# awslabs/dgl-ke

Measured on AMD Instinct MI355X. Metric: positive edges/sec (whole node), higher is better.
Workload: dtype f32

## Files before the change

dgl-ke_amd/csrc/kge_api.hip:

```cpp
#include <cmath>
#include <cstdarg>
#include <cstdio>
#include <cstring>
#include <new>
#include <algorithm>
#include "kge_common.hpp"
#include "kge_sampler_common.hpp"

namespace {

thread_local char g_err[512] = "";

int fail(int code, const char *fmt, ...) {
    va_list ap;
    va_start(ap, fmt);
    vsnprintf(g_err, sizeof(g_err), fmt, ap);
    va_end(ap);
    return code;
}

#define KGE_TRY(expr)                                                                  \
    do {                                                                               \
        const int rc_ = (expr);                                                        \
        if (rc_ != KGE_OK) return fail(rc_, "%s failed (%d) at %s:%d", #expr, rc_, __FILE__, __LINE__); \
// ... 211 lines not shown
        na.S = out;
        KGE_TRY(launch_neg_fwd_pair(na, s));
    }
    return KGE_OK;
}

int kge_score_neg_bwd(int model, int neg_head, const float *pos_side, const float *rel, const float *neg, const float *neg_score,
                      const float *dneg, int C, int chunk, int N, int d_e, int d_r, float gamma, float emb_init, float *g_pos_side,
                      float *g_rel, float *g_neg, void *ws, size_t ws_bytes, unsigned flags, void *stream) {
    if (int rc = check_model(model, d_e, d_r)) return rc;
    if (!pos_side || !rel || !neg || !dneg || !g_pos_side || !g_rel || !g_neg || !ws || C < 0 || chunk <= 0 || N <= 0)
        return fail(KGE_ERR_ARG, "kge_score_neg_bwd: bad argument");
    if (model == KGE_TRANSR) return no_modular_transr();
    if ((model == KGE_TRANSE_L2 || model == KGE_SIMPLE) && !neg_score)
        return fail(KGE_ERR_ARG, "kge_score_neg_bwd: TransE_l2 / SimplE need the forward scores");
    if (C == 0) return KGE_OK;
    hipStream_t s = (hipStream_t)stream;
    const int B = C * chunk;
    Carver cv(ws, ws_bytes); NegBufs w;
    const size_t need = carve_neg(cv, w, model, C, chunk, N, d_e);
    if (need > ws_bytes) return fail(KGE_ERR_WORKSPACE, "workspace too small: need %zu bytes", need);
    if (int rc = neg_prepare(model, neg_head, pos_side, rel, neg, C, chunk, N, d_e, d_r, gamma, emb_init, false, w, s)) return rc;
    const float *Wuse = dneg;
    if (model == KGE_TRANSE_L2 || model == KGE_SIMPLE) {
        const int64_t n = (int64_t)B * N;
        const dim3 grid((unsigned)((n + 255) / 256));
        if (model == KGE_TRANSE_L2) hipLaunchKernelGGL(l2_scale_kernel, grid, dim3(256), 0, s, dneg, neg_score, gamma, w.W, n);
        else hipLaunchKernelGGL(clamp_mask_kernel, grid, dim3(256), 0, s, dneg, neg_score, KGE_SIMPLE_CLAMP, w.W, n);
        Wuse = w.W;
    }
    bool gemm = use_mfma(model, d_e, N, flags);
    if (gemm) {
        GemmArgs g; fill_gemm(g, model, C, chunk, N, d_e, gamma, w.A, neg, nullptr);
        g.W = Wuse; g.GA = w.GA; g.GN = g_neg;
        const int rc = launch_neg_bwd_gemm(g, s);
        if (rc == KGE_ERR_ARG) gemm = false;
        else if (rc != KGE_OK) return fail(rc, "launch_neg_bwd_gemm failed (%d)", rc);
    }
    if (!gemm) {
        NegArgs na; fill_pair(na, model, C, chunk, N, d_e, gamma, w.A, neg, nullptr);
        na.W = Wuse; na.GA = w.GA; na.GN = g_neg;
        na.GNp = (flags & KGE_FLAG_TWO_PASS_PAIR) ? nullptr : w.GNp;
        KGE_TRY(launch_neg_bwd_pair(na, s));
    }
    if (model == KGE_RESCAL) {
        RescalMatvecArgs m{};
        m.B = B; m.D = d_e; m.rel = rel; m.z1 = w.GA; m.c1 = g_pos_side;
        KGE_TRY(launch_rescal_matvec(m, s));
        RescalOuterArgs o{};
        o.B = B; o.D = d_e; o.u = w.GA; o.v = pos_side; o.G = g_rel;
        KGE_TRY(launch_rescal_outer(o, s));
        return KGE_OK;
    }
    EdgeBwdArgs e;
    fill_edge_bwd(e, EdgeSrc{pos_side, nullptr, pos_side, nullptr, rel, nullptr}, model, B, d_e, d_r, neg_head, gamma,
                  rot_div_of(emb_init), nullptr, w.GA);
    e.GH = neg_head ? nullptr : g_pos_side;
    e.GT = neg_head ? g_pos_side : nullptr;
    e.GR = g_rel;
    KGE_TRY(launch_edge_bwd(e, s));
    return KGE_OK;
}

int kge_loss_fwd_bwd(int loss_genre, int adv, float adv_temp, int pairwise, float margin, const float *pos, const float *neg,
                     const float *w, int64_t B, int N, float *loss3, float *dpos, float *dneg, void *ws, size_t ws_bytes, void *stream) {
    if (int rc = check_loss(loss_genre, adv, pairwise)) return rc;
    if (!pos || !neg || !dpos || !dneg || !ws || B <= 0 || N <= 0)
// ... 386 lines not shown
    if (p.fold_loss) {
        LossArgs la; fill_step_loss(la); la.skip_pos = 1;
        KGE_TRY(launch_neg_fwd_gemm_with_edge_loss(g, ef, la, out->tickets, s));
    } else KGE_TRY(launch_neg_fwd_gemm_with_edge(g, ef, s, c.tail));
    return KGE_OK;
}

int Step::phase_fwd() {
    if (p.transr) {
    } else if (p.gemm) {
        if (int rc = fwd_gemm()) return rc;
    } else {
        if (c.co_update) KGE_TRY(launch_update(*c.co_update, s));
        if (p.merged_pair) {
            NegArgs nf = na;
            nf.nbase = tb->ent; nf.nidx = b->neg_ids;
            nf.xbase = tb->ent; nf.xidx = b->neg_head ? b->t_gid : b->h_gid; nf.rbase = tb->rel; nf.ridx = b->rel_ids;
            nf.asign = b->neg_head ? -1.f : 1.f;
            KGE_TRY(launch_neg_fwd_bcast_with_edge(nf, ef, s));
        } else KGE_TRY(launch_neg_fwd_pair(na, s));
    }
    if (p.fused_loss || p.fold_loss) return KGE_OK;
    LossArgs la; fill_step_loss(la);
    la.row_pos = p.want4 ? w.row_pos : nullptr;
    if (p.merged_fwd && p.is_l2) { la.l2_raw = 1; la.l2_chunk = b->chunk; la.asq = w.asq; la.bsq = w.bsq; }
    la.skip_pos = (p.pairwise || p.rescal || p.transr) ? 0 : 1; la.diag_chunk = p.nd ? b->chunk : 0;
    KGE_TRY(launch_loss(la, s));
    return KGE_OK;
}

int Step::bwd_neg_gemm() {
    g.W = w.S; g.w = b->edge_w; g.lp = lp;
    if (p.dense_bwd) { g.nbase = w.Bn; g.nidx = nullptr; }
    g.GA = w.GA; g.GN = GN;
    if (p.qfuse) {
        g.Q = w.GT; g.QP = w.GH; g.qc = b->neg_head ? 1.f : -1.f;
        if (!(out && out->g_rel)) g.GA = nullptr;
    }
    g.reg_coef = (p.reg && !p.nd) ? hp->reg_coef : 0.f; g.reg_norm = hp->reg_norm;
    g.row_neg = (p.fused_loss && p.want4) ? w.row_neg : nullptr;
    g.acc = p.fused_loss ? acc : nullptr;
    if (p.ew_bwd) {
        g.ew_ent = src.hbase; g.ew_rel = src.rbase; g.ew_h = src.hidx; g.ew_t = src.tidx; g.ew_r = src.ridx;
        g.ew_dpos = w.dP; g.ew_GH = w.GH; g.ew_GT = w.GT; g.ew_GR = GR;
        g.ew_reg_coef = p.reg ? hp->reg_coef : 0.f; g.ew_reg_norm = hp->reg_norm; g.ew_neg_head = b->neg_head;
        if (!(out && out->g_rel)) g.GA = nullptr;
    }
    if (c.co_prep) {
        const int rc = launch_neg_bwd_gemm_with_prep(g, *c.co_prep, s);
        if (rc == KGE_OK) return KGE_OK;
        if (rc != KGE_ERR_ARG) return fail(rc, "launch_neg_bwd_gemm_with_prep failed (%d)", rc);
    }
    KGE_TRY(launch_neg_bwd_gemm(g, s, c.tail));
    if (c.co_prep) KGE_TRY(launch_edge_fwd(*c.co_prep, s));
    return KGE_OK;
}

int Step::bwd_transr() {
    const int B = b->B, d_e = hp->d_e;
    KGE_TRY(launch_transr_bwd(tr, s));
    RescalMatvecArgs m{};
    m.B = B; m.D = d_e; m.Dc = hp->d_r; m.rel = tbx->proj; m.ridx = b->rel_ids;
    m.y1 = tr.SG; m.r1 = w.TR1; m.y2 = tr.DQ; m.r2 = w.TR2;
    KGE_TRY(launch_rescal_matvec(m, s));
    KGE_TRY(launch_rescal_axpy(w.dP, w.TR1, b->neg_head ? nullptr : w.TR2, B, d_e, w.GH, s, -1.f));
    KGE_TRY(launch_rescal_axpy(w.dP, w.TR1, b->neg_head ? w.TR2 : nullptr, B, d_e, w.GT, s, 1.f));
    if (p.nd) KGE_TRY(launch_nd_fold(GN, b->neg_head ? w.GH : w.GT, B, b->chunk, p.N, d_e, s));
// ... 693 lines not shown
```

dgl-ke_amd/csrc/kge_common.hpp:

```cpp
#pragma once
#include <hip/hip_runtime.h>
#include <stdint.h>
#include "../../include/kge_hip.h"

#define KGE_WAVE 64
#define KGE_BLOCK 256
#define KGE_WAVES_PER_BLOCK (KGE_BLOCK / KGE_WAVE)

typedef float f32x4 __attribute__((ext_vector_type(4)));


#ifdef KGE_TIMELINE
#define KGE_TL_PER_KERNEL 8192
static __device__ unsigned long long *kge_tl_buf = nullptr;
__device__ __forceinline__ void kge_tl_mark(int kid, int n) {
    asm volatile("s_waitcnt vmcnt(0) lgkmcnt(0)" ::: "memory");
    const int wid = (int)(blockIdx.x * (blockDim.x >> 6) + (threadIdx.x >> 6));
    if ((threadIdx.x & 63) == 0 && kge_tl_buf && wid < KGE_TL_PER_KERNEL)
        kge_tl_buf[((size_t)kid * KGE_TL_PER_KERNEL + wid) * 8 + 4 + n] = wall_clock64();
}
struct KgeTlScope {
    unsigned long long t0; int kid; int wid;
    __device__ __forceinline__ KgeTlScope(int kid_, int wid_) : kid(kid_), wid(wid_) { t0 = wall_clock64(); }
    __device__ __forceinline__ void mark(int n) { kge_tl_mark(kid, n); }
// ... 374 lines not shown
bool rank_gemm_supported(int model, int d_e);
size_t rank_gemm_mask_bytes(int rows, int64_t N);
int launch_rank_gemm(int model, const float *A, int rows, const float *nbase, const int64_t *nidx, int64_t N, int D, float gamma,
                     float clampv, const float *asq, const float *bsq, const float *P, void *mask, const int64_t *filt_ptr,
                     const int64_t *filt_ids, int64_t e0, int32_t *ranks, hipStream_t s);
struct ChunkCands {
    const int64_t *cand; int64_t n_cand, stride;
    const int64_t *own;
    int64_t n_ent, E; int chunk;
};
int launch_chunk_bsq(const ChunkCands &cc, int64_t c0, int rows, int64_t n_list, const float *ent, int D, float *bsq_own, float *bsq_c,
                     hipStream_t s);
int launch_rank_chunk_gemm(int model, const ChunkCands &cc, int64_t c0, int nch, const float *A, const float *asq, const float *P,
                           const float *ent, int D, float gamma, float clampv, const float *bsq_own, const float *bsq_c, int shared,
                           const int64_t *filt_ptr, const int64_t *filt_ids, int32_t *ranks, hipStream_t s);
int launch_chunk_ids(const ChunkCands &cc, int64_t cfirst, int nch, int m, int64_t ncols, int64_t *ids, hipStream_t s);
int launch_chunk_count(const ChunkCands &cc, int64_t cfirst, int nch, int m, int64_t ncols, const float *S, const float *P,
                       const int64_t *filt_ptr, const int64_t *filt_ids, int32_t *ranks, hipStream_t s);
int launch_rel_query(int model, const float *ent, const int64_t *h, const int64_t *t, int rows, int d_e, float *Q, float *qsq,
                     hipStream_t s);
int launch_rel_rotate_score(const float *ent, const float *rel, const int64_t *h, const int64_t *t, int rows, int64_t n_rel, int d_e,
                            float gamma, float rot_div, float *S, hipStream_t s);
int launch_rel_neg_rows(const float *rel, int64_t n_rel, int d_r, float *out, int64_t *ids, int64_t n_ids, hipStream_t s);
int launch_rel_count_t(const float *St, const float *P, int rows, int64_t N, const int64_t *filt_ptr, const int64_t *filt_ids,
                       int64_t e0, int32_t *ranks, hipStream_t s);
struct GemmArgs {
    int model, C, chunk, N, D;
    float gamma;
    const float *A;
    const float *nbase; const int64_t *nidx;
    const float *asq, *bsq;
    const float *xbase; const int64_t *xidx; const float *rbase; const int64_t *ridx; float asign;
    int lds_off;
    float *S;
    float clampv;
    float *PM, *PS, *PL;
    float *Sraw;
    float adv_temp;
    const float *W;
    const float *w;
    LossParams lp; int B;
    float *GA, *GN;
    float *Q; const float *QP; float qc;
    const float *ew_ent, *ew_rel; const int64_t *ew_h, *ew_t, *ew_r; const float *ew_dpos;
    float *ew_GH, *ew_GT, *ew_GR; float ew_reg_coef; int ew_reg_norm, ew_neg_head;
    float reg_coef; int reg_norm;
    float *row_neg;
    float *acc;
};
bool neg_mfma_supported(int model, int d_e, int N);
bool neg_gemm_fused_loss_supported(int chunk, int N);
int launch_neg_fwd_gemm(const GemmArgs &a, hipStream_t s);
int launch_neg_bwd_gemm(const GemmArgs &a, hipStream_t s, const SmpTail *tail = nullptr);
struct UpdateArgs;
int launch_neg_fwd_gemm_with_update(const GemmArgs &a, const UpdateArgs &u, hipStream_t s);
bool neg_fwd_gemm_with_edge_supported(int model, int d_e, int d_r);
int launch_neg_fwd_gemm_with_edge(const GemmArgs &a, const EdgeFwdArgs &e, hipStream_t s, const SmpTail *tail = nullptr);
struct LossArgs;
bool neg_fwd_loss_fold_supported(int model, int C, int chunk, int N, int d_e, int d_r);
int launch_neg_fwd_gemm_with_edge_loss(const GemmArgs &a, const EdgeFwdArgs &e, const LossArgs &la, int *tickets, hipStream_t s);
int launch_neg_bwd_gemm_with_prep(const GemmArgs &a, const EdgeFwdArgs &e, hipStream_t s);
int launch_neg_fwd_pair(const NegArgs &a, hipStream_t s);
int launch_neg_bwd_pair(const NegArgs &a, hipStream_t s);
struct RescalMatvecArgs {
    int B, D;
    int Dc;
// ... 91 lines not shown
```

dgl-ke_amd/csrc/kge_neg_gemm.hip:

```cpp
#include "kge_common.hpp"
#include "kge_update_body.hpp"
#include "kge_edge_fwd_body.hpp"
#include "kge_sampler_tail.hpp"
#include "kge_loss_body.hpp"

using namespace kge;
KGE_TL_DEFINE(gemm)

#define MFMA16(a, b, c) __builtin_amdgcn_mfma_f32_16x16x4f32((a), (b), (c), 0, 0, 0)
#define KGE_PIN_ACC(x, y) do { asm volatile("" : "+a"(x), "+a"(y) :: "memory"); __builtin_amdgcn_sched_barrier(0); } while (0)
#define KGE_ORDER() do { asm volatile("" ::: "memory"); __builtin_amdgcn_sched_barrier(0); } while (0)

bool neg_mfma_supported(int model, int d_e, int N) {
    (void)N;
    if (model != KGE_TRANSE_L2 && model != KGE_DISTMULT && model != KGE_COMPLEX && model != KGE_SIMPLE &&
        model != KGE_RESCAL) return false;
    return d_e % 4 == 0;
}

bool neg_gemm_fused_loss_supported(int chunk, int N) { return N <= 256 && chunk <= 768; }

static inline int check_launch_g() { return hipGetLastError() == hipSuccess ? KGE_OK : KGE_ERR_LAUNCH; }
__device__ __forceinline__ float4 ldg4(const float *p) { return *reinterpret_cast<const float4 *>(p); }
__device__ __forceinline__ float4 zero4() { return make_float4(0.f, 0.f, 0.f, 0.f); }
// ... 621 lines not shown
#pragma unroll
    for (int k = 0; k < GB_TJ; ++k) {
        const bool ok = k < tj;
        vm[k] = (ok && a.lp.adv) ? pm[k] : -INFINITY;
        vs[k] = (ok && a.lp.adv) ? ps[k] : 0.f;
        vl[k] = (LOSS && ok) ? pl[k] : 0.f;
    }
    if (!a.lp.adv) {
        M = 0.f; coef = base / (float)a.N;
        if (LOSS) {
            float l = 0.f;
#pragma unroll
            for (int k = 0; k < GB_TJ; ++k) l += vl[k];
            lrow = 2.f * coef * l;
        }
        if (fac) for (int k = 0; k < tj; ++k) fac[k] = coef;
        return;
    }
    float mx = vm[0];
#pragma unroll
    for (int k = 1; k < GB_TJ; ++k) mx = fmaxf(mx, vm[k]);
    float z = 0.f, l = 0.f, e[GB_TJ];
#pragma unroll
    for (int k = 0; k < GB_TJ; ++k) { e[k] = __expf(vm[k] - mx); z += vs[k] * e[k]; if (LOSS) l += vl[k] * e[k]; }
    M = mx; coef = base / z;
    if (LOSS) lrow = 2.f * coef * l;
    if (fac) {
#pragma unroll
        for (int k = 0; k < GB_TJ; ++k) if (k < tj) fac[k] = e[k] * coef;
    }
}
#define GB_TJP 17

template <bool L2, bool FACT, bool ISGA, bool DENSE = false, int KS = 1, int EW = 0>
__device__ __forceinline__ void neg_bwd_gemm_tile(const GemmArgs &a, int ti, int tj, int td, int c, int bcl, int maxK,
                                                  float *smem) {
    const int lane = threadIdx.x & 63, wv = (threadIdx.x >> 6) & (KGE_WAVES_PER_BLOCK - 1);
    const int kh = KS == 1 ? 0 : (int)(threadIdx.x >> 6) / KGE_WAVES_PER_BLOCK;
    constexpr bool isGA = ISGA;
    const int tl0 = bcl * KGE_WAVES_PER_BLOCK + wv;
    const int tr = isGA ? ti : tj;
    constexpr bool PAIRED = EW >= 2 && ISGA;
    if (PAIRED) td = (a.D / 2 + 31) / 32;
    const bool tile_ok = tl0 < tr * td;
    const int tl = KS == 1 ? tl0 : min(tl0, tr * td - 1);
    const int dt = tl % td, rt = tl / td;
    const int D = a.D, N = a.N, chunk = a.chunk;
    const int m = lane & 15, q = lane >> 4;
    const int K = isGA ? N : chunk;
    const int R = isGA ? chunk : N;

    const int Kc = a.D / 2;
    const int dre = dt * 32 + (m & 7) * 4;
    const int d = PAIRED ? (m < 8 ? dre : Kc + dre) : dt * 64 + m * 4;
    const bool dok = PAIRED ? dre < Kc : d < D;
    const int dc = dok ? d : 0;
    int64_t *rix = reinterpret_cast<int64_t *>(smem);
    float *ftab = smem + 2 * maxK;
    const int k0 = threadIdx.x;
    const int64_t rbase = isGA ? (int64_t)c * N : (int64_t)c * chunk;
    int64_t rix0 = 0;
    if (!DENSE) {
        if (isGA) rix0 = a.nidx ? a.nidx[(int64_t)c * N + min(k0, K - 1)] : (int64_t)c * N + k0;
        else rix0 = (int64_t)c * chunk + k0;
    }
    const bool need_self = L2 || ((!isGA) && a.reg_coef > 0.f && a.reg_norm > 0);
    const bool wantQ = isGA && a.Q != nullptr;
    float4 selfv[4], pq[4];
    int64_t srow[4];
#pragma unroll
    for (int r = 0; r < 4; ++r) { selfv[r] = zero4(); pq[r] = zero4(); srow[r] = (int64_t)c * R + min(rt * 16 + q * 4 + r, R - 1); }
    int64_t ewh[4], ewt[4], ewr[4];
    float ewdp[4];
    if constexpr (EW && ISGA) {
#pragma unroll
        for (int r = 0; r < 4; ++r) {
            ewh[r] = a.ew_h[srow[r]]; ewt[r] = a.ew_t[srow[r]]; ewr[r] = a.ew_r[srow[r]];
            ewdp[r] = a.ew_dpos ? a.ew_dpos[srow[r]] : 0.f;
        }
    }
    if (isGA) {
        if (L2) {
#pragma unroll
            for (int r = 0; r < 4; ++r) selfv[r] = ldg4(a.A + srow[r] * D + dc);
        }
        const float *qp = a.QP + dc;
#pragma unroll
        for (int r = 0; r < 4; ++r) pq[r] = ldg4(qp + srow[r] * D);
    } else if (!DENSE && need_self && a.nidx) {
#pragma unroll
        for (int r = 0; r < 4; ++r) srow[r] = a.nidx[srow[r]];
    }
    if (!DENSE) {
        if (k0 < K) rix[k0] = rix0;
        for (int k = k0 + KS * KGE_BLOCK; k < K; k += KS * KGE_BLOCK)
            rix[k] = isGA ? (a.nidx ? a.nidx[(int64_t)c * N + k] : (int64_t)c * N + k) : (int64_t)c * chunk + k;
    }
    if (FACT && !isGA) {
        for (int k = threadIdx.x; k < K; k += KS * KGE_BLOCK) {
            float M, coef, lr;
            row_stats<false>(a, (int64_t)c * chunk + k, tj, M, coef, lr, ftab + k * GB_TJP);
        }
    }
    float rM = 0.f, rcoef = 0.f;
    const float *PMrow = FACT ? a.PM : nullptr;
    if (FACT && isGA) {
        const int rowg = min(rt * 16 + m, chunk - 1);
        const int64_t gi = (int64_t)c * chunk + rowg;
        const bool do_loss = dt == 0 && kh == 0 && (a.row_neg || a.acc);
        float lrow = 0.f;
        if (do_loss) row_stats<true>(a, gi, tj, rM, rcoef, lrow);
        else row_stats<false>(a, gi, tj, rM, rcoef, lrow);
        PMrow = a.PM + gi * tj;
        if (do_loss && q == 0 && tile_ok && rt * 16 + m < chunk) {
            if (a.row_neg) a.row_neg[gi] = lrow;
            if (a.acc) {
                const int slot = (int)(gi & (KGE_ACC_SLOTS - 1));
                atomicAdd(a.acc + 1 * KGE_ACC_SLOTS + slot, lrow);
                atomicAdd(a.acc + 2 * KGE_ACC_SLOTS + slot, 0.5f * lrow);
            }
        }
    }
    if (!DENSE) __syncthreads();
    if (KS == 1 && !tile_ok) return;
    const float *ft = ftab + rt;

    const float *Wc = a.W + (int64_t)c * chunk * N;
    const float *Ac = a.A + (int64_t)c * chunk * D;
    const int row = rt * 16 + m;
    const bool rok = row < R;
    const int rowc = min(row, R - 1);
    const bool vecW = isGA && (N % 4 == 0);
    const float *Wrow = isGA ? Wc + (int64_t)rowc * N : Wc + rowc;
    const int64_t wstride = isGA ? 1 : N;
    f32x4 acc[4];
#pragma unroll
    for (int s_ = 0; s_ < 4; ++s_) acc[s_] = (f32x4){0.f, 0.f, 0.f, 0.f};
    float wsum = 0.f;
    BwdStage s0[BU], s1[BU];

    const int msall = K >> 4;
    const int mlo = KS == 1 ? 0 : kh * (msall / KS);
    const int msfull = (KS == 1 || kh == KS - 1) ? msall : (kh + 1) * (msall / KS);
    const float *Xb = (isGA ? a.nbase : a.A) + dc;
    const float *Wq = Wrow + (int64_t)(q * 4) * wstride;

#define BWD_LOAD(ST, MS0, VECW)                                                                \
    _Pragma("unroll") for (int u = 0; u < BU; ++u) {                                           \
        const int ms = min((MS0) + u, msfull - 1);                                             \
        int64_t ri[4];                                                                         \
        _Pragma("unroll") for (int e = 0; e < 4; ++e)                                          \
            ri[e] = DENSE ? rbase + (ms * 16 + q * 4 + e) : rix[ms * 16 + q * 4 + e];          \
        if (VECW) {                                                                            \
            const float4 t4 = ldg4(Wq + ms * 16);                                              \
            ST[u].w[0] = t4.x; ST[u].w[1] = t4.y; ST[u].w[2] = t4.z; ST[u].w[3] = t4.w;        \
        } else {                                                                               \
            _Pragma("unroll") for (int e = 0; e < 4; ++e)                                      \
                ST[u].w[e] = Wq[(int64_t)(ms * 16 + e) * wstride];                             \
        }                                                                                      \
        if (FACT) ST[u].pm = PMrow[isGA ? ms : 0];         \
        _Pragma("unroll") for (int e = 0; e < 4; ++e) ST[u].r[e] = ldg4(Xb + ri[e] * D);       \
    }
#define BWD_XFORM(ST, MS0)                                                                     \
    if (FACT) {                                                                                \
        _Pragma("unroll") for (int u = 0; u < BU; ++u) {                                       \
            const int ms = min((MS0) + u, msfull - 1);                                         \
            if (isGA) {                                                                        \
                const float f_ = a.lp.adv ? __expf(ST[u].pm - rM) * rcoef : rcoef;             \
                _Pragma("unroll") for (int e = 0; e < 4; ++e) ST[u].w[e] *= f_;               \
            } else {                                                                           \
                _Pragma("unroll") for (int e = 0; e < 4; ++e)                                  \
                    ST[u].w[e] *= ft[(ms * 16 + q * 4 + e) * GB_TJP];                          \
            }                                                                                  \
        }                                                                                      \
    }
#define BWD_MMA1(ST, u)                                                                        \
    _Pragma("unroll") for (int e = 0; e < 4; ++e) {                                            \
        const float wgt = ST[u].w[e];                                                          \
        wsum += wgt;                                                                           \
        acc[0] = MFMA16(wgt, ST[u].r[e].x, acc[0]);                                            \
        acc[1] = MFMA16(wgt, ST[u].r[e].y, acc[1]);                                            \
        acc[2] = MFMA16(wgt, ST[u].r[e].z, acc[2]);                                            \
        acc[3] = MFMA16(wgt, ST[u].r[e].w, acc[3]);                                            \
    }
#define BWD_MMA(ST) _Pragma("unroll") for (int u = 0; u < BU; ++u) { BWD_MMA1(ST, u) }
#define BWD_MMA_G(ST, MS0) _Pragma("unroll") for (int u = 0; u < BU; ++u) { if ((MS0) + u < msfull) { BWD_MMA1(ST, u) } }
#define BWD_PIPE(VECW)                                                                         \
    {                                                                                          \
        BWD_LOAD(s0, mlo, VECW);                                                               \
        int g = mlo;                                                                           \
        for (; g + 2 * BU <= msfull; g += 2 * BU) {                                            \
            BWD_LOAD(s1, g + BU, VECW);                                                        \
            KGE_ORDER();                            \
            BWD_XFORM(s0, g);                                                                  \
            BWD_MMA(s0);                                                                       \
            KGE_ORDER();                                                                       \
            BWD_LOAD(s0, g + 2 * BU, VECW);                                                    \
            KGE_ORDER();                                                                       \
            BWD_XFORM(s1, g + BU);                                                             \
            BWD_MMA(s1);                                                                       \
            KGE_ORDER();                                                                       \
        }                                                                                      \
        if (g < msfull) {                              \
            BWD_LOAD(s1, g + BU, VECW);                                                        \
            BWD_XFORM(s0, g);                                                                  \
            BWD_MMA_G(s0, g);                                                                  \
            BWD_XFORM(s1, g + BU);                                                             \
            BWD_MMA_G(s1, g + BU);                                                             \
        }                                                                                      \
    }

    const bool has_tail = (K & 15) != 0;
    float tw[4];
    float4 tx[4];
    float tpm = 0.f;
    {
        const int kk = msall * 16 + q * 4;
#pragma unroll
        for (int e = 0; e < 4; ++e) {
            const int kc = min(kk + e, K - 1);
            tw[e] = Wrow[(int64_t)kc * wstride];
            tx[e] = ldg4(Xb + (DENSE ? rbase + kc : rix[kc]) * D);
        }
        if (FACT && isGA) tpm = PMrow[min(msall, tj - 1)];
    }
    if (!isGA && need_self) {
#pragma unroll
        for (int r = 0; r < 4; ++r) selfv[r] = ldg4(a.nbase + srow[r] * D + dc);
    }
    float4 ehv[4], etv[4], erv[4];
    if constexpr (EW && ISGA) {
#pragma unroll
        for (int r = 0; r < 4; ++r) {
            ehv[r] = ldg4(a.ew_ent + ewh[r] * D + dc); etv[r] = ldg4(a.ew_ent + ewt[r] * D + dc);
            erv[r] = ldg4(a.ew_rel + ewr[r] * D + dc);
        }
    }
    KGE_TL_MARK_K(3, 0);
    if (msfull > mlo) {
        if (isGA && vecW) BWD_PIPE(true) else BWD_PIPE(false)
    }
    KGE_TL_MARK_K(3, 1);
#undef BWD_LOAD
#undef BWD_XFORM
#undef BWD_MMA1
#undef BWD_MMA
#undef BWD_MMA_G
#undef BWD_PIPE
    if (has_tail && kh == KS - 1) {
        const int kk = msall * 16 + q * 4;
        float ftail = 1.f;
        if (FACT && isGA) ftail = a.lp.adv ? __expf(tpm - rM) * rcoef : rcoef;
#pragma unroll
        for (int e = 0; e < 4; ++e) {
// ... 114 lines not shown
            }
            if constexpr (EW == 1 && ISGA) {
                const float dp = ewdp[r];
                const float gx[4] = {o.x, o.y, o.z, o.w};
                const float hh[4] = {ehv[r].x, ehv[r].y, ehv[r].z, ehv[r].w}, tt[4] = {etv[r].x, etv[r].y, etv[r].z, etv[r].w};
                const float rr[4] = {erv[r].x, erv[r].y, erv[r].z, erv[r].w};
                Pack<4> gh, gt, gr;
#pragma unroll
                for (int e = 0; e < 4; ++e) {
                    float o_h = dp * rr[e] * tt[e], o_r = dp * hh[e] * tt[e], o_t = dp * hh[e] * rr[e];
                    if (a.ew_neg_head) { o_t += gx[e] * rr[e]; o_r += gx[e] * tt[e]; }
                    else               { o_h += gx[e] * rr[e]; o_r += gx[e] * hh[e]; }
                    if (a.ew_reg_coef > 0.f && a.ew_reg_norm > 0) {
                        if (a.ew_reg_norm == 3) o_r += reg_grad3(rr[e], a.ew_reg_coef);
                        else o_r += reg_grad(rr[e], a.ew_reg_coef, a.ew_reg_norm);
                    }
                    gh.v[e] = o_h; gt.v[e] = o_t; gr.v[e] = o_r;
                }
                const int64_t eo = ((int64_t)c * R + ro) * D + d;
                if (a.ew_GH) st_wt<4>(a.ew_GH + eo, gh);
                if (a.ew_GT) st_wt<4>(a.ew_GT + eo, gt);
                st_wt<4>(a.ew_GR + eo, gr);
            }
            if (wantQ) {
                Pack<4> qv;
                qv.v[0] = o.x + a.qc * pq[r].x; qv.v[1] = o.y + a.qc * pq[r].y;
                qv.v[2] = o.z + a.qc * pq[r].z; qv.v[3] = o.w + a.qc * pq[r].w;
                st_wt<4>(a.Q + ((int64_t)c * R + ro) * D + d, qv);
            }
        }
    }
}

template <bool L2, bool FACT, bool DENSE = false, int KS = 1, int EW = 0>
__device__ __forceinline__ void neg_bwd_gemm_body(const GemmArgs &a, int ti, int tj, int td, int bpA, int bpN, int maxK,
                                                  int bid, int nblk, float *smem) {
    const int blk = xcd_remap(bid, nblk);
    const int c = blk / (bpA + bpN);
    const int bc = blk % (bpA + bpN);
    if (bc < bpA) neg_bwd_gemm_tile<L2, FACT, true, DENSE, KS, EW>(a, ti, tj, td, c, bc, maxK, smem);
    else neg_bwd_gemm_tile<L2, FACT, false, DENSE, KS, 0>(a, ti, tj, td, c, bc - bpA, maxK, smem);
}

#define GB_KS 1
template <bool L2, bool FACT, bool DENSE = false, int EW = 0>
__global__ __launch_bounds__(GB_KS * KGE_BLOCK) void neg_bwd_gemm_kernel(const int64_t *nidx, const float *A, const float *qp, int toff, int nbM,
                                                                         int bpA, int bpN, int chunk, int N, int D, int maxK,
                                                                         GemmArgs a_in, SmpTail st) {
    extern __shared__ __attribute__((aligned(16))) float smem[];
    if ((int)blockIdx.x < toff) {
        if constexpr (GB_KS == 1) sampler_tail_p2(st, (int)blockIdx.x);
        return;
    }
    KGE_TL(3);
    GemmArgs a = a_in;
    a.nidx = nidx; a.A = A; a.QP = qp; a.chunk = chunk; a.N = N; a.D = D;
    const int ti = (chunk + 15) / 16, tj = (N + 15) / 16, td = (D + 63) / 64;
    neg_bwd_gemm_body<L2, FACT, DENSE, GB_KS, EW>(a, ti, tj, td, bpA, bpN, maxK, (int)blockIdx.x - toff, nbM, smem);
}

template <bool L2, int MODEL>
__global__ __launch_bounds__(KGE_BLOCK) void neg_bwd_prep_kernel(GemmArgs a, int ti, int tj, int td, int bpA, int bpN,
                                                                 int maxK, int nbG, EdgeFwdArgs e) {
    extern __shared__ __attribute__((aligned(16))) float smem[];
    if ((int)blockIdx.x < nbG) {
        KGE_TL(3);
        neg_bwd_gemm_body<L2, false, true>(a, ti, tj, td, bpA, bpN, maxK, (int)blockIdx.x, nbG, smem);
    } else {
        KGE_TL(0);
        edge_fwd_body<MODEL, 4, false>(e, (int)blockIdx.x - nbG);
    }
}

int launch_neg_bwd_gemm(const GemmArgs &a, hipStream_t s, const SmpTail *tail) {
    if (a.C == 0) return tail && tail->phase ? KGE_ERR_ARG : KGE_OK;
    SmpTail st{};
    if (tail && tail->phase && GB_KS == 1) { st = *tail; st.phase = 2; }
    const int nbT = st.phase ? 8 : 0;
    if (!a.W) return KGE_ERR_ARG;
    const bool fact = a.PM != nullptr;
    if (fact && (a.lp.pairwise || !a.PS || !a.PL)) return KGE_ERR_ARG;
    const int maxK = a.chunk > a.N ? a.chunk : a.N;
    if (maxK > GB_MAXK) return KGE_ERR_ARG;
    const int ti = (a.chunk + 15) / 16, tj = (a.N + 15) / 16, td = (a.D + 63) / 64;
    const int bpA = (ti * td + KGE_WAVES_PER_BLOCK - 1) / KGE_WAVES_PER_BLOCK;
    const int bpN = (tj * td + KGE_WAVES_PER_BLOCK - 1) / KGE_WAVES_PER_BLOCK;
    const int nb = a.C * (bpA + bpN);
    const int mk = (maxK + 3) & ~3;
    if (fact && !neg_gemm_fused_loss_supported(a.chunk, a.N)) return KGE_ERR_ARG;
    const size_t sm = (size_t)mk * 8 + (fact ? (size_t)mk * GB_TJP * 4 : 0);
    const bool l2 = a.model == KGE_TRANSE_L2;
    const dim3 g(nb + nbT), b(GB_KS * KGE_BLOCK);
#define KGE_BG_H(BPA_, NB_) a.nidx, a.A, (a.Q ? a.QP : a.A), nbT, NB_, BPA_, bpN, a.chunk, a.N, a.D, mk, a, st
    if (a.ew_GR) {
        const bool simple = a.model == KGE_SIMPLE, cplx = a.model == KGE_COMPLEX || simple;
        if (fact || l2 || (a.model != KGE_DISTMULT && !cplx) || !a.ew_ent || !a.ew_rel || !a.ew_h || !a.ew_t || !a.ew_r ||
            a.D % (cplx ? 8 : 4))
            return KGE_ERR_ARG;
        if (cplx) {
            const int tdA = (a.D / 2 + 31) / 32;
            const int bpAc = (ti * tdA + KGE_WAVES_PER_BLOCK - 1) / KGE_WAVES_PER_BLOCK;
            const int nbc = a.C * (bpAc + bpN);
            const dim3 gc(nbc + nbT);
            if (simple) {
                if (!a.nidx) hipLaunchKernelGGL((neg_bwd_gemm_kernel<false, false, true, 3>), gc, b, 0, s, KGE_BG_H(bpAc, nbc));
                else hipLaunchKernelGGL((neg_bwd_gemm_kernel<false, false, false, 3>), gc, b, sm, s, KGE_BG_H(bpAc, nbc));
            } else if (!a.nidx) hipLaunchKernelGGL((neg_bwd_gemm_kernel<false, false, true, 2>), gc, b, 0, s, KGE_BG_H(bpAc, nbc));
            else hipLaunchKernelGGL((neg_bwd_gemm_kernel<false, false, false, 2>), gc, b, sm, s, KGE_BG_H(bpAc, nbc));
            return check_launch_g();
        }
        if (!a.nidx) hipLaunchKernelGGL((neg_bwd_gemm_kernel<false, false, true, 1>), g, b, 0, s, KGE_BG_H(bpA, nb));
        else hipLaunchKernelGGL((neg_bwd_gemm_kernel<false, false, false, 1>), g, b, sm, s, KGE_BG_H(bpA, nb));
        return check_launch_g();
    }
    if (!fact && !a.nidx) {
        if (l2) hipLaunchKernelGGL((neg_bwd_gemm_kernel<true, false, true>), g, b, 0, s, KGE_BG_H(bpA, nb));
        else hipLaunchKernelGGL((neg_bwd_gemm_kernel<false, false, true>), g, b, 0, s, KGE_BG_H(bpA, nb));
        return check_launch_g();
    }
    if (l2 && fact) hipLaunchKernelGGL((neg_bwd_gemm_kernel<true, true>), g, b, sm, s, KGE_BG_H(bpA, nb));
    else if (l2) hipLaunchKernelGGL((neg_bwd_gemm_kernel<true, false>), g, b, sm, s, KGE_BG_H(bpA, nb));
    else if (fact) hipLaunchKernelGGL((neg_bwd_gemm_kernel<false, true>), g, b, sm, s, KGE_BG_H(bpA, nb));
    else hipLaunchKernelGGL((neg_bwd_gemm_kernel<false, false>), g, b, sm, s, KGE_BG_H(bpA, nb));
    return check_launch_g();
}
#undef KGE_BG_H

int launch_neg_fwd_gemm_with_update(const GemmArgs &a, const UpdateArgs &u, hipStream_t s) {
    if (a.C == 0 || a.PM) return KGE_ERR_ARG;
    const int dmax = u.model_d_e > u.d_r ? u.model_d_e : u.d_r;
    const bool inplace = !u.emit_ent && !u.emit_rel && !u.g0 && !u.g1 && !u.gs0 && !u.gs1 && !u.gr && !u.gsr && !u.rid &&
                         !u.dry && !u.nd_chunk && u.em.n == 0 && u.rm.n == 0;
    if (!inplace || u.model_d_e % 4 || u.d_r % 4 || dmax > 1024) return KGE_ERR_ARG;
    if (u.reg_coef > 0.f && u.reg_norm > 0 && u.reg_norm != 3) return KGE_ERR_ARG;
    const int nbE = (u.UE + KGE_WAVES_PER_BLOCK - 1) / KGE_WAVES_PER_BLOCK, nbR = (u.UR + KGE_WAVES_PER_BLOCK - 1) / KGE_WAVES_PER_BLOCK;
    if (nbE + nbR == 0) return KGE_ERR_ARG;
    const int ti = (a.chunk + 15) / 16, tj = (a.N + 15) / 16;
    const int64_t ntiles = (int64_t)a.C * ti * tj;
    const int nbG = (int)((ntiles + KGE_WAVES_PER_BLOCK - 1) / KGE_WAVES_PER_BLOCK);
    const bool l2 = a.model == KGE_TRANSE_L2;
    const int nit = dmax <= 256 ? 1 : (dmax <= 512 ? 2 : 4);
    if (u.transe_fast && !u.Q) return KGE_ERR_ARG;
    const int lean = u.transe_fast ? 3 : 2;
    const dim3 g(nbG + nbE + nbR), b(KGE_BLOCK);
#define KGE_FU(L2_, N_, LE_) hipLaunchKernelGGL((neg_fwd_update_kernel<L2_, N_, LE_>), g, b, 0, s, a, ti, tj, nbG, u, nbE)
#define KGE_FU_N(N_) do { if (l2) { if (lean == 3) KGE_FU(true, N_, 3); else KGE_FU(true, N_, 2); }           \
                          else { if (lean == 3) return KGE_ERR_ARG; KGE_FU(false, N_, 2); } } while (0)
    if (nit == 1) KGE_FU_N(1); else if (nit == 2) KGE_FU_N(2); else KGE_FU_N(4);
#undef KGE_FU_N
#undef KGE_FU
// ... 35 lines not shown
```

dgl-ke_amd/dglke_amd/_lib.py:

```python
import contextlib
import ctypes as C
import gc
import os
import threading

import torch

_HERE = os.path.dirname(os.path.abspath(__file__))
LIB_PATH = os.environ.get("KGE_LIB") or os.path.join(_HERE, "libkge_hip.so")

KGE_ABI_VERSION = 8
MODEL_IDS = {"TransE_l1": 0, "TransE_l2": 1, "TransE": 1, "DistMult": 2, "ComplEx": 3, "RotatE": 4, "SimplE": 5, "RESCAL": 6, "TransR": 7}
LOSS_IDS = {"Logsigmoid": 0, "Logistic": 1, "Hinge": 2, "BCE": 3}
FLAG_FORCE_PAIRWISE = 1
FLAG_NO_TRANSE_FAST = 2
FLAG_DENSE_NEG = 4
FLAG_FUSED_LOSS = 8
FLAG_TWO_PASS_PAIR = 16
FLAG_NEG_DEG_SAMPLE = 32
FLAG_ASYNC_REL = 64
FLAG_DENSE_BWD = 256
FLAG_FWD_DIRECT = 512
FLAG_LOSS_IN_FWD = 1024
TICKET_INTS = 4096
FLAG_SPLIT_FWD = 128
PHASE_GATHER, PHASE_FORWARD, PHASE_BACKWARD, PHASE_UPDATE = 1, 2, 4, 8
ACC_SLOTS = 4096

c_f = C.c_float
c_i = C.c_int
c_i32 = C.c_int32
c_i64 = C.c_int64
c_p = C.c_void_p
c_sz = C.c_size_t
c_u = C.c_uint


class KgeBatch(C.Structure):
    _fields_ = [("B", c_i32), ("C", c_i32), ("chunk", c_i32), ("N", c_i32), ("neg_head", c_i32),
                ("U", c_i32), ("UE", c_i32), ("UR", c_i32),
                ("h_gid", c_p), ("t_gid", c_p), ("rel_ids", c_p), ("neg_ids", c_p), ("edge_w", c_p),
                ("ue_id", c_p), ("ue_pos_ptr", c_p), ("ue_pos_adj", c_p), ("ue_neg_ptr", c_p),
                ("ue_neg_slot", c_p), ("ur_id", c_p), ("ur_ptr", c_p), ("ur_edge", c_p),
                ("ue_rec", c_p), ("ur_rec", c_p), ("counts_dev", c_p),
                ("edge_w_mean", c_f), ("reserved_", c_i32)]


class KgeHParams(C.Structure):
    _fields_ = [("model", c_i32), ("d_e", c_i32), ("d_r", c_i32), ("loss_genre", c_i32),
                ("adv", c_i32), ("pairwise", c_i32), ("reg_norm", c_i32), ("flags", C.c_uint32),
                ("gamma", c_f), ("emb_init", c_f), ("lr", c_f), ("adv_temp", c_f), ("margin", c_f),
                ("reg_coef", c_f), ("eps", c_f)]


class KgeTables(C.Structure):
    _fields_ = [("ent", c_p), ("ent_state", c_p), ("rel", c_p), ("rel_state", c_p),
# ... 245 lines not shown
```

include/kge_hip.h:

```cpp
#ifndef KGE_HIP_H
#define KGE_HIP_H

#include <stddef.h>
#include <stdint.h>

#ifdef __cplusplus
extern "C" {
#endif

#define KGE_ABI_VERSION 8

enum kge_model {
    KGE_TRANSE_L1 = 0,
    KGE_TRANSE_L2 = 1,
    KGE_DISTMULT  = 2,
    KGE_COMPLEX   = 3,
    KGE_ROTATE    = 4,
    KGE_TRANSR    = 7,
    KGE_RESCAL    = 6,
    KGE_SIMPLE    = 5
};

enum kge_loss {
    KGE_LOSS_LOGSIGMOID = 0,
    KGE_LOSS_LOGISTIC   = 1,
    KGE_LOSS_HINGE      = 2,
    KGE_LOSS_BCE        = 3
};

enum kge_status {
    KGE_OK            = 0,
    KGE_ERR_ARG       = -1,
    KGE_ERR_WORKSPACE = -2,
    KGE_ERR_LAUNCH    = -3
};

#define KGE_FLAG_FORCE_PAIRWISE 1u
#define KGE_FLAG_NO_TRANSE_FAST 2u
#define KGE_FLAG_DENSE_NEG 4u
#define KGE_FLAG_FUSED_LOSS 8u
#define KGE_FLAG_TWO_PASS_PAIR 16u
#define KGE_FLAG_NEG_DEG_SAMPLE 32u
#define KGE_FLAG_ASYNC_REL 64u

#define KGE_FLAG_SPLIT_FWD 128u

#define KGE_FLAG_DENSE_BWD 256u

#define KGE_FLAG_FWD_DIRECT 512u

#define KGE_FLAG_LOSS_IN_FWD 1024u

int         kge_abi_version(void);
const char *kge_last_error(void);

int kge_gather_rows(const float *table, int64_t n_rows, int dim, const int64_t *idx,
                    int64_t n_idx, float *out, void *stream);

int kge_score_pos(int model, const float *h, const float *r, const float *t, int64_t B, int d_e,
                  int d_r, float gamma, float emb_init, float *out, void *stream);
int kge_score_pos_bwd(int model, const float *h, const float *r, const float *t,
                      const float *dpos, int64_t B, int d_e, int d_r, float gamma,
                      float emb_init, float *gh, float *gr, float *gt, void *stream);

size_t kge_score_neg_workspace_bytes(int model, int C, int chunk, int N, int d_e);
int kge_score_neg_fwd(int model, int neg_head, const float *pos_side, const float *rel,
                      const float *neg, int C, int chunk, int N, int d_e, int d_r, float gamma,
                      float emb_init, float *out, void *ws, size_t ws_bytes, unsigned flags,
                      void *stream);
int kge_score_neg_bwd(int model, int neg_head, const float *pos_side, const float *rel,
                      const float *neg, const float *neg_score, const float *dneg, int C,
                      int chunk, int N, int d_e, int d_r, float gamma, float emb_init,
                      float *g_pos_side, float *g_rel, float *g_neg, void *ws, size_t ws_bytes,
                      unsigned flags, void *stream);

int kge_loss_fwd_bwd(int loss_genre, int adv, float adv_temp, int pairwise, float margin,
                     const float *pos, const float *neg, const float *w, int64_t B, int N,
                     float *loss3, float *dpos, float *dneg, void *ws, size_t ws_bytes,
                     void *stream);

int kge_adagrad_scatter(float *table, float *state_sum, int64_t n_rows, int dim,
                        const int64_t *idx, const float *grad, int64_t n_idx, float lr, float eps,
                        void *stream);

// ... 250 lines not shown
```

Baseline: 33.80 million.

## Stage backward GEMM weight tile in LDS instead of per-k global loads

In the negative-sample backward GEMM, the weight/score matrix W is now cooperatively loaded into shared memory once per block, transposed for the GN path, before the k-loop. The k-loop then reads W from LDS rather than issuing strided global loads each iteration. The aim is to cut uncoalesced global traffic and latency in the backward pass. This costs extra LDS capacity, which can lower occupancy, plus staging registers. It is enabled by default when the shape fits in 64KB and can be turned off with a new flag.

```diff
diff --git a/dgl-ke_amd/csrc/kge_api.hip b/dgl-ke_amd/csrc/kge_api.hip
--- a/dgl-ke_amd/csrc/kge_api.hip
+++ b/dgl-ke_amd/csrc/kge_api.hip
@@ -267,7 +267,7 @@
     bool gemm = use_mfma(model, d_e, N, flags);
     if (gemm) {
         GemmArgs g; fill_gemm(g, model, C, chunk, N, d_e, gamma, w.A, neg, nullptr);
-        g.W = Wuse; g.GA = w.GA; g.GN = g_neg;
+        g.W = Wuse; g.GA = w.GA; g.GN = g_neg; g.wlds_off = (flags & KGE_FLAG_BWD_W_DIRECT) ? 1 : 0;
         const int rc = launch_neg_bwd_gemm(g, s);
         if (rc == KGE_ERR_ARG) gemm = false;
         else if (rc != KGE_OK) return fail(rc, "launch_neg_bwd_gemm failed (%d)", rc);
@@ -720,7 +720,7 @@
 int Step::bwd_neg_gemm() {
     g.W = w.S; g.w = b->edge_w; g.lp = lp;
     if (p.dense_bwd) { g.nbase = w.Bn; g.nidx = nullptr; }
-    g.GA = w.GA; g.GN = GN;
+    g.GA = w.GA; g.GN = GN; g.wlds_off = (hp->flags & KGE_FLAG_BWD_W_DIRECT) ? 1 : 0;
     if (p.qfuse) {
         g.Q = w.GT; g.QP = w.GH; g.qc = b->neg_head ? 1.f : -1.f;
         if (!(out && out->g_rel)) g.GA = nullptr;
diff --git a/dgl-ke_amd/csrc/kge_common.hpp b/dgl-ke_amd/csrc/kge_common.hpp
--- a/dgl-ke_amd/csrc/kge_common.hpp
+++ b/dgl-ke_amd/csrc/kge_common.hpp
@@ -430,6 +430,7 @@
     const float *asq, *bsq;
     const float *xbase; const int64_t *xidx; const float *rbase; const int64_t *ridx; float asign;
     int lds_off;
+    int wlds_off;
     float *S;
     float clampv;
     float *PM, *PS, *PL;
diff --git a/dgl-ke_amd/csrc/kge_neg_gemm.hip b/dgl-ke_amd/csrc/kge_neg_gemm.hip
--- a/dgl-ke_amd/csrc/kge_neg_gemm.hip
+++ b/dgl-ke_amd/csrc/kge_neg_gemm.hip
@@ -677,7 +677,9 @@
 }
 #define GB_TJP 17
 
-template <bool L2, bool FACT, bool ISGA, bool DENSE = false, int KS = 1, int EW = 0>
+#define GB_WL_GA 0
+#define GB_WSLOTS 7
+template <bool L2, bool FACT, bool ISGA, bool DENSE = false, int KS = 1, int EW = 0, bool WL = false>
 __device__ __forceinline__ void neg_bwd_gemm_tile(const GemmArgs &a, int ti, int tj, int td, int c, int bcl, int maxK,
                                                   float *smem) {
     const int lane = threadIdx.x & 63, wv = (threadIdx.x >> 6) & (KGE_WAVES_PER_BLOCK - 1);
@@ -709,6 +711,27 @@
         if (isGA) rix0 = a.nidx ? a.nidx[(int64_t)c * N + min(k0, K - 1)] : (int64_t)c * N + k0;
         else rix0 = (int64_t)c * chunk + k0;
     }
+    float *Ws = smem + 2 * maxK;
+    const int KP = ((K + 15) & ~15) + 4;
+    const int rtA = (bcl * KGE_WAVES_PER_BLOCK) / td;
+    const int nwb = min(bcl * KGE_WAVES_PER_BLOCK + KGE_WAVES_PER_BLOCK - 1, tr * td - 1) / td - rtA + 1;
+    const int K4 = K >> 2;
+    const int wtot = WL ? (isGA ? nwb * 16 * K4 : K * nwb * 4) : 0;
+    const float winv = 1.f / (float)(isGA ? K4 : nwb * 4);
+    float4 wst[GB_WSLOTS];
+    if constexpr (WL) {
+        const float *Wc0 = a.W + (int64_t)c * chunk * N;
+        const int wlast = min(nwb * 16, chunk - rtA * 16) * K4 - 1;
+#pragma unroll
+        for (int j = 0; j < GB_WSLOTS; ++j) {
+            const int i = (int)threadIdx.x + j * KGE_BLOCK;
+            if (isGA) wst[j] = ldg4(Wc0 + (int64_t)rtA * 16 * N + (int64_t)min(i, wlast) * 4);
+            else {
+                const int k = (int)(((float)i + 0.5f) * winv), p = i - k * (nwb * 4);
+                wst[j] = ldg4(Wc0 + (int64_t)min(k, K - 1) * N + min(rtA * 16 + p * 4, N - 4));
+            }
+        }
+    }
     const bool need_self = L2 || ((!isGA) && a.reg_coef > 0.f && a.reg_norm > 0);
     const bool wantQ = isGA && a.Q != nullptr;
     float4 selfv[4], pq[4];
@@ -740,6 +763,31 @@
         if (k0 < K) rix[k0] = rix0;
         for (int k = k0 + KS * KGE_BLOCK; k < K; k += KS * KGE_BLOCK)
             rix[k] = isGA ? (a.nidx ? a.nidx[(int64_t)c * N + k] : (int64_t)c * N + k) : (int64_t)c * chunk + k;
+    }
+    if constexpr (WL) {
+        auto wput = [&](int i, const float4 &v) {
+            if (i >= wtot) return;
+            const int k = (int)(((float)i + 0.5f) * winv);
+            if (isGA) {
+                *reinterpret_cast<float4 *>(Ws + k * KP + (i - k * K4) * 4) = v;
+            } else {
+                float *wd = Ws + (i - k * (nwb * 4)) * 4 * KP + k;
+                wd[0] = v.x; wd[KP] = v.y; wd[2 * KP] = v.z; wd[3 * KP] = v.w;
+            }
+        };
+#pragma unroll
+        for (int j = 0; j < GB_WSLOTS; ++j) wput((int)threadIdx.x + j * KGE_BLOCK, wst[j]);
+        const float *Wc0 = a.W + (int64_t)c * chunk * N;
+        const int wlast = min(nwb * 16, chunk - rtA * 16) * K4 - 1;
+        for (int i = (int)threadIdx.x + GB_WSLOTS * KGE_BLOCK; i < wtot; i += KGE_BLOCK) {
+            float4 v;
+            if (isGA) v = ldg4(Wc0 + (int64_t)rtA * 16 * N + (int64_t)min(i, wlast) * 4);
+            else {
+                const int k = (int)(((float)i + 0.5f) * winv), p = i - k * (nwb * 4);
+                v = ldg4(Wc0 + (int64_t)min(k, K - 1) * N + min(rtA * 16 + p * 4, N - 4));
+            }
+            wput(i, v);
+        }
     }
     if (FACT && !isGA) {
         for (int k = threadIdx.x; k < K; k += KS * KGE_BLOCK) {
@@ -789,6 +837,7 @@
     const int msfull = (KS == 1 || kh == KS - 1) ? msall : (kh + 1) * (msall / KS);
     const float *Xb = (isGA ? a.nbase : a.A) + dc;
     const float *Wq = Wrow + (int64_t)(q * 4) * wstride;
+    const float *Wsq = Ws + ((rt - rtA) * 16 + m) * KP + q * 4;
 
 #define BWD_LOAD(ST, MS0, VECW)                                                                \
     _Pragma("unroll") for (int u = 0; u < BU; ++u) {                                           \
@@ -796,7 +845,10 @@
         int64_t ri[4];                                                                         \
         _Pragma("unroll") for (int e = 0; e < 4; ++e)                                          \
             ri[e] = DENSE ? rbase + (ms * 16 + q * 4 + e) : rix[ms * 16 + q * 4 + e];          \
-        if (VECW) {                                                                            \
+        if (WL) {                                                                              \
+            const float4 t4 = *reinterpret_cast<const float4 *>(Wsq + ms * 16);                \
+            ST[u].w[0] = t4.x; ST[u].w[1] = t4.y; ST[u].w[2] = t4.z; ST[u].w[3] = t4.w;        \
+        } else if (VECW) {                                                                     \
             const float4 t4 = ldg4(Wq + ms * 16);                                              \
             ST[u].w[0] = t4.x; ST[u].w[1] = t4.y; ST[u].w[2] = t4.z; ST[u].w[3] = t4.w;        \
         } else {                                                                               \
@@ -861,10 +913,14 @@
     float tpm = 0.f;
     {
         const int kk = msall * 16 + q * 4;
+        if constexpr (WL) {
+            const float4 t4 = *reinterpret_cast<const float4 *>(Wsq + min(msall * 16, KP - 4 - q * 4));
+            tw[0] = t4.x; tw[1] = t4.y; tw[2] = t4.z; tw[3] = t4.w;
+        }
 #pragma unroll
         for (int e = 0; e < 4; ++e) {
             const int kc = min(kk + e, K - 1);
-            tw[e] = Wrow[(int64_t)kc * wstride];
+            if constexpr (!WL) tw[e] = Wrow[(int64_t)kc * wstride];
             tx[e] = ldg4(Xb + (DENSE ? rbase + kc : rix[kc]) * D);
         }
         if (FACT && isGA) tpm = PMrow[min(msall, tj - 1)];
@@ -1045,18 +1101,18 @@
     }
 }
 
-template <bool L2, bool FACT, bool DENSE = false, int KS = 1, int EW = 0>
+template <bool L2, bool FACT, bool DENSE = false, int KS = 1, int EW = 0, bool WL = false>
 __device__ __forceinline__ void neg_bwd_gemm_body(const GemmArgs &a, int ti, int tj, int td, int bpA, int bpN, int maxK,
                                                   int bid, int nblk, float *smem) {
     const int blk = xcd_remap(bid, nblk);
     const int c = blk / (bpA + bpN);
     const int bc = blk % (bpA + bpN);
-    if (bc < bpA) neg_bwd_gemm_tile<L2, FACT, true, DENSE, KS, EW>(a, ti, tj, td, c, bc, maxK, smem);
-    else neg_bwd_gemm_tile<L2, FACT, false, DENSE, KS, 0>(a, ti, tj, td, c, bc - bpA, maxK, smem);
+    if (bc < bpA) neg_bwd_gemm_tile<L2, FACT, true, DENSE, KS, EW, WL && GB_WL_GA>(a, ti, tj, td, c, bc, maxK, smem);
+    else neg_bwd_gemm_tile<L2, FACT, false, DENSE, KS, 0, WL>(a, ti, tj, td, c, bc - bpA, maxK, smem);
 }
 
 #define GB_KS 1
-template <bool L2, bool FACT, bool DENSE = false, int EW = 0>
+template <bool L2, bool FACT, bool DENSE = false, int EW = 0, bool WL = false>
 __global__ __launch_bounds__(GB_KS * KGE_BLOCK) void neg_bwd_gemm_kernel(const int64_t *nidx, const float *A, const float *qp, int toff, int nbM,
                                                                          int bpA, int bpN, int chunk, int N, int D, int maxK,
                                                                          GemmArgs a_in, SmpTail st) {
@@ -1069,7 +1125,7 @@
     GemmArgs a = a_in;
     a.nidx = nidx; a.A = A; a.QP = qp; a.chunk = chunk; a.N = N; a.D = D;
     const int ti = (chunk + 15) / 16, tj = (N + 15) / 16, td = (D + 63) / 64;
-    neg_bwd_gemm_body<L2, FACT, DENSE, GB_KS, EW>(a, ti, tj, td, bpA, bpN, maxK, (int)blockIdx.x - toff, nbM, smem);
+    neg_bwd_gemm_body<L2, FACT, DENSE, GB_KS, EW, WL>(a, ti, tj, td, bpA, bpN, maxK, (int)blockIdx.x - toff, nbM, smem);
 }
 
 template <bool L2, int MODEL>
@@ -1104,6 +1160,11 @@
     const size_t sm = (size_t)mk * 8 + (fact ? (size_t)mk * GB_TJP * 4 : 0);
     const bool l2 = a.model == KGE_TRANSE_L2;
     const dim3 g(nb + nbT), b(GB_KS * KGE_BLOCK);
+    const bool pairedA = a.ew_GR && (a.model == KGE_COMPLEX || a.model == KGE_SIMPLE);
+    auto wblocks = [](int t) { return t == 1 ? 4 : (t % KGE_WAVES_PER_BLOCK == 0 ? 1 : 2); };
+    const int nwbA = GB_WL_GA ? wblocks(pairedA ? (a.D / 2 + 31) / 32 : td) : 0, nwbN = wblocks(td);
+    const size_t smw = (size_t)mk * 8 + (size_t)(nwbA > nwbN ? nwbA : nwbN) * 16 * (((maxK + 15) & ~15) + 4) * 4;
+    const bool wl = GB_KS == 1 && !fact && a.nidx && !a.wlds_off && a.N % 4 == 0 && smw <= 64 * 1024;
 #define KGE_BG_H(BPA_, NB_) a.nidx, a.A, (a.Q ? a.QP : a.A), nbT, NB_, BPA_, bpN, a.chunk, a.N, a.D, mk, a, st
     if (a.ew_GR) {
         const bool simple = a.model == KGE_SIMPLE, cplx = a.model == KGE_COMPLEX || simple;
@@ -1117,18 +1178,26 @@
             const dim3 gc(nbc + nbT);
             if (simple) {
                 if (!a.nidx) hipLaunchKernelGGL((neg_bwd_gemm_kernel<false, false, true, 3>), gc, b, 0, s, KGE_BG_H(bpAc, nbc));
+                else if (wl) hipLaunchKernelGGL((neg_bwd_gemm_kernel<false, false, false, 3, true>), gc, b, smw, s, KGE_BG_H(bpAc, nbc));
                 else hipLaunchKernelGGL((neg_bwd_gemm_kernel<false, false, false, 3>), gc, b, sm, s, KGE_BG_H(bpAc, nbc));
             } else if (!a.nidx) hipLaunchKernelGGL((neg_bwd_gemm_kernel<false, false, true, 2>), gc, b, 0, s, KGE_BG_H(bpAc, nbc));
+            else if (wl) hipLaunchKernelGGL((neg_bwd_gemm_kernel<false, false, false, 2, true>), gc, b, smw, s, KGE_BG_H(bpAc, nbc));
             else hipLaunchKernelGGL((neg_bwd_gemm_kernel<false, false, false, 2>), gc, b, sm, s, KGE_BG_H(bpAc, nbc));
             return check_launch_g();
         }
         if (!a.nidx) hipLaunchKernelGGL((neg_bwd_gemm_kernel<false, false, true, 1>), g, b, 0, s, KGE_BG_H(bpA, nb));
+        else if (wl) hipLaunchKernelGGL((neg_bwd_gemm_kernel<false, false, false, 1, true>), g, b, smw, s, KGE_BG_H(bpA, nb));
         else hipLaunchKernelGGL((neg_bwd_gemm_kernel<false, false, false, 1>), g, b, sm, s, KGE_BG_H(bpA, nb));
         return check_launch_g();
     }
     if (!fact && !a.nidx) {
         if (l2) hipLaunchKernelGGL((neg_bwd_gemm_kernel<true, false, true>), g, b, 0, s, KGE_BG_H(bpA, nb));
         else hipLaunchKernelGGL((neg_bwd_gemm_kernel<false, false, true>), g, b, 0, s, KGE_BG_H(bpA, nb));
+        return check_launch_g();
+    }
+    if (wl) {
+        if (l2) hipLaunchKernelGGL((neg_bwd_gemm_kernel<true, false, false, 0, true>), g, b, smw, s, KGE_BG_H(bpA, nb));
+        else hipLaunchKernelGGL((neg_bwd_gemm_kernel<false, false, false, 0, true>), g, b, smw, s, KGE_BG_H(bpA, nb));
         return check_launch_g();
     }
     if (l2 && fact) hipLaunchKernelGGL((neg_bwd_gemm_kernel<true, true>), g, b, sm, s, KGE_BG_H(bpA, nb));
diff --git a/dgl-ke_amd/dglke_amd/_lib.py b/dgl-ke_amd/dglke_amd/_lib.py
--- a/dgl-ke_amd/dglke_amd/_lib.py
+++ b/dgl-ke_amd/dglke_amd/_lib.py
@@ -22,6 +22,7 @@
 FLAG_DENSE_BWD = 256
 FLAG_FWD_DIRECT = 512
 FLAG_LOSS_IN_FWD = 1024
+FLAG_BWD_W_DIRECT = 2048
 TICKET_INTS = 4096
 FLAG_SPLIT_FWD = 128
 PHASE_GATHER, PHASE_FORWARD, PHASE_BACKWARD, PHASE_UPDATE = 1, 2, 4, 8
diff --git a/include/kge_hip.h b/include/kge_hip.h
--- a/include/kge_hip.h
+++ b/include/kge_hip.h
@@ -50,6 +50,8 @@
 #define KGE_FLAG_FWD_DIRECT 512u
 
 #define KGE_FLAG_LOSS_IN_FWD 1024u
+
+#define KGE_FLAG_BWD_W_DIRECT 2048u
 
 int         kge_abi_version(void);
 const char *kge_last_error(void);
```

Result: no change. 33.68 million (-0.4%).
